# marcin-ochman/modular-slam

Measured on AMD Instinct MI355X. Metric: ORB keypoints extracted+matched /sec, 640×480 RGB-D, 1/2/4/8 GPU; HBM GB/s vs roofline, higher is better.
Workload: dtype u8

## Files before the change

modular-slam_amd/csrc/k_fast.hip:

```cpp
#include <type_traits>
#include "common.hpp"
#include "arc_score.hpp"

namespace mslam
{

constexpr int kTileP = 80;
constexpr int kTileX = 1;
constexpr int kScP = 68;

__device__ __forceinline__ CellDesc load_cell(const CellDesc* __restrict__ cells, int cell)
{
    typedef uint32_t u32x4_t __attribute__((ext_vector_type(4)));
    u32x4_t r;
    const uint32_t off = (uint32_t)cell * (uint32_t)sizeof(CellDesc);
    asm volatile("s_load_dwordx4 %0, %1, %2\n\ts_waitcnt lgkmcnt(0)" : "=s"(r) : "s"(cells), "s"(off));
    CellDesc c;
    c.level = (int16_t)(r.x & 0xFFFFu), c.cw = (int16_t)(r.x >> 16);
    c.ch = (int16_t)(r.y & 0xFFFFu), c.pad = 0;
    c.x0 = (int16_t)(r.z & 0xFFFFu), c.y0 = (int16_t)(r.z >> 16);
    c.ox = (int16_t)(r.w & 0xFFFFu), c.oy = (int16_t)(r.w >> 16);
    return c;
}
static_assert(sizeof(CellDesc) == 16, "load_cell reads a descriptor as four dwords");

__device__ __forceinline__ int min3i(int a, int b, int c) { return min(min(a, b), c); }
__device__ __forceinline__ int max3i(int a, int b, int c) { return max(max(a, b), c); }

__global__ __launch_bounds__(256) __attribute__((amdgpu_waves_per_eu(8, 8))) void k_fast_cells(const uint8_t* __restrict__ pyr, Geometry g,
                                                    const CellDesc* __restrict__ cells, uint32_t* __restrict__ cell_cnt,
                                                    uint32_t* __restrict__ cell_kp, int ini_thr, int min_thr, int n_frames)
{
    __shared__ __attribute__((aligned(16))) uint8_t tile[70 * kTileP];
    __shared__ __attribute__((aligned(16))) uint8_t sc[(66 * kScP + 15) / 16 * 16];
    __shared__ __attribute__((aligned(4))) uint16_t cand[64 * 64];
    __shared__ uint32_t bitmap[64 * 2];
    constexpr uint32_t kPassCap = 512;
    __shared__ uint16_t plist[kPassCap];
    __shared__ uint32_t n_cand, n_pass;

    const bool spread = n_frames < 8;
    const int xcd = blockIdx.x & 7, cell_id = spread ? (int)blockIdx.x : (int)(blockIdx.x >> 3);
    const int f_local = spread ? (int)blockIdx.y : (int)blockIdx.y * 8 + xcd;
    if(f_local >= n_frames)
        return;
    const size_t frame = (size_t)f_local + g.frame0;
    const CellDesc c = load_cell(cells, cell_id);
    const LevelGeom& lv = g.lv[c.level];
    const int cw = c.cw, ch = c.ch;
    const int tid = threadIdx.x, lane = tid & 63, wave = tid >> 6;

    {
        const uint8_t* src = pyr + frame * g.slab + lv.offset + (size_t)c.y0 * lv.pitch + (c.x0 - kTileX);
        const int n_chunks = ch * 5;
#pragma unroll
        for(int p = 0; p < 2; ++p)
        {
            const int t = p * 256 + tid;
            if(t < n_chunks)
            {
                const int r = (t * 13108) >> 16, j = t - r * 5;
                const uint32_t off = (uint32_t)(r * lv.pitch + 16 * j);
                __builtin_amdgcn_global_load_lds(
                    (const __attribute__((address_space(1))) void*)(src + off),
                    (__attribute__((address_space(3))) void*)&tile[(p * 256 + wave * 64) * 16], 16, 0, 0);
            }
        }
    }
    if(tid < (66 * kScP + 15) / 16 - 256)
        reinterpret_cast<uint4*>(sc)[256 + tid] = make_uint4(0u, 0u, 0u, 0u);
    if(tid < 128)
        bitmap[tid] = 0;
    if(tid == 0)
        n_cand = 0, n_pass = 0;
    __builtin_amdgcn_s_waitcnt(0x0F70);
    __syncthreads();

    const uint32_t n_cand_lds = (uint32_t)(size_t)(__attribute__((address_space(3))) void*)(&n_cand);
    const uint32_t n_pass_lds = (uint32_t)(size_t)(__attribute__((address_space(3))) void*)(&n_pass);
    uint32_t total = 0;
    for(int pass = 0; pass < 2; ++pass)
    {
        const int thr = pass == 0 ? ini_thr : min_thr;

        {
            typedef __attribute__((address_space(3))) uint32_t* lds32_t;
            typedef __attribute__((address_space(3))) uint16_t* lds16_t;
            typedef uint32_t u32x4_t __attribute__((ext_vector_type(4)));
            typedef __attribute__((address_space(3))) u32x4_t* lds128_t;
            uint32_t t_op = threadIdx.x;
            asm volatile("" : "+v"(t_op));
            const uint32_t ln = t_op & 63u;
            const int wv = __builtin_amdgcn_readfirstlane((int)(t_op >> 6));
            const int ngrp = (cw - 6 + 3) >> 2;
            const int lg = ngrp > 8 ? 4 : ngrp > 4 ? 3 : ngrp > 2 ? 2 : ngrp > 1 ? 1 : 0;
            const int i4 = (int)(ln & ((1u << lg) - 1u)), sub = (int)(ln >> lg);
            const int rps = 64 >> lg;
            const int n_steps = (ch - 6 + rps - 1) >> (6 - lg);
            const int tq = min(max(thr, 0), 254);
            const uint32_t kb = (uint32_t)(256 - ((tq + 256) >> 1)) * 0x01010101u;
            const uint32_t kd = (uint32_t)(255 - ((254 - tq) >> 1)) * 0x01010101u;
            const int xl = 3 + 4 * i4;
            const int n_col = min(max(cw - 3 - xl, 0), 4);
            const uint32_t colmask = (uint32_t)(0x80808080ull >> (8 * (4 - n_col)));
            const uint32_t tile_lds = (uint32_t)(size_t)(__attribute__((address_space(3))) void*)tile;
            const uint32_t cand_lds = (uint32_t)(size_t)(__attribute__((address_space(3))) void*)cand;
            const uint32_t seg_lds = (uint32_t)(size_t)(__attribute__((address_space(3))) void*)sc + (uint32_t)wv * 1024u;
            int y = 3 + wv * rps + sub;
            uint32_t row = tile_lds + (uint32_t)((y - 3) * kTileP + 4 * i4);
            uint32_t yx = (uint32_t)((y << 8) | xl);
            uint32_t n_grp = 0;
            auto steps = [&](auto checked) {
                constexpr bool CHECKED = decltype(checked)::value;
#pragma unroll 1
                for(int st = wv; st < n_steps; st += 4, y += CHECKED ? 4 * rps : 0, row += (uint32_t)(4 * rps * kTileP), yx += (uint32_t)(4 * rps) << 8)
                {
                    uint32_t keep = 0;
                    if(!CHECKED || (colmask != 0 && y < ch - 3))
                    {
                        const lds32_t r = lds_ptr<lds32_t>(row);
                        const uint32_t d0 = r[60], d1 = r[61], d2 = r[62];
                        const uint32_t nC = ~d1, U = r[1], D = r[121];
                        const uint32_t Lf = __builtin_amdgcn_alignbyte(d1, d0, 1);
                        const uint32_t Rt = __builtin_amdgcn_alignbyte(d2, d1, 3);
                        const uint32_t q0 = __builtin_amdgcn_lerp(D, nC, 0u), q8 = __builtin_amdgcn_lerp(U, nC, 0u);
                        const uint32_t q4 = __builtin_amdgcn_lerp(Rt, nC, 0u), q12 = __builtin_amdgcn_lerp(Lf, nC, 0u);
                        const uint32_t br = (__builtin_amdgcn_lerp(q0, kb, 0u) | __builtin_amdgcn_lerp(q8, kb, 0u)) &
                                            (__builtin_amdgcn_lerp(q4, kb, 0u) | __builtin_amdgcn_lerp(q12, kb, 0u));
                        const uint32_t nd = (__builtin_amdgcn_lerp(q0, kd, 0u) & __builtin_amdgcn_lerp(q8, kd, 0u)) |
                                            (__builtin_amdgcn_lerp(q4, kd, 0u) & __builtin_amdgcn_lerp(q12, kd, 0u));
                        keep = (br | ~nd) & (CHECKED ? colmask : 0x80808080u);
                    }
                    const bool any = keep != 0;
                    const unsigned long long vote = __ballot(any);
                    if(any)
                        lds_ptr<lds32_t>(seg_lds)[n_grp + __builtin_amdgcn_mbcnt_hi((uint32_t)(vote >> 32), __builtin_amdgcn_mbcnt_lo((uint32_t)vote, 0u))] =
                            keep | yx;
                    n_grp += (uint32_t)__popcll(vote);
                }
            };
            if(cw == 70 && ch == 70)
                steps(std::false_type{});
            else
                steps(std::true_type{});
            for(uint32_t i0 = 0; i0 < n_grp; i0 += 64)
            {
                const uint32_t rec = i0 + ln < n_grp ? lds_ptr<lds32_t>(seg_lds)[i0 + ln] : 0u;
                const bool f0 = (rec & 0x80u) != 0, f1 = (rec & 0x8000u) != 0, f2 = (rec & 0x800000u) != 0, f3 = (int)rec < 0;
                const unsigned long long m0 = __ballot(f0), m1 = __ballot(f1), m2 = __ballot(f2), m3 = __ballot(f3);
                const uint32_t c0 = (uint32_t)__popcll(m0), c1 = (uint32_t)__popcll(m1), c2 = (uint32_t)__popcll(m2),
                               c3 = (uint32_t)__popcll(m3);
                uint32_t base;
                {
                    uint32_t got;
                    unsigned long long save;
                    const uint32_t add = c0 + c1 + c2 + c3;
                    asm volatile("s_mov_b64 %1, exec\n\t"
                                 "s_mov_b64 exec, 1\n\t"
                                 "ds_add_rtn_u32 %0, %2, %3\n\t"
                                 "s_waitcnt lgkmcnt(0)\n\t"
                                 "s_mov_b64 exec, %1"
                                 : "=&v"(got), "=&s"(save)
                                 : "v"(n_cand_lds), "v"(add)
                                 : "memory");
                    base = (uint32_t)__builtin_amdgcn_readfirstlane((int)got);
                }
                const uint32_t v = rec & 0x7F7Fu;
                uint32_t b2 = cand_lds + 2u * base;
                if(f0)
                    *lds_ptr<lds16_t>(b2 + 2u * __builtin_amdgcn_mbcnt_hi((uint32_t)(m0 >> 32), __builtin_amdgcn_mbcnt_lo((uint32_t)m0, 0u))) = (uint16_t)v;
                b2 += 2u * c0;
                if(f1)
                    *lds_ptr<lds16_t>(b2 + 2u * __builtin_amdgcn_mbcnt_hi((uint32_t)(m1 >> 32), __builtin_amdgcn_mbcnt_lo((uint32_t)m1, 0u))) = (uint16_t)(v + 1);
                b2 += 2u * c1;
                if(f2)
                    *lds_ptr<lds16_t>(b2 + 2u * __builtin_amdgcn_mbcnt_hi((uint32_t)(m2 >> 32), __builtin_amdgcn_mbcnt_lo((uint32_t)m2, 0u))) = (uint16_t)(v + 2);
                b2 += 2u * c2;
                if(f3)
                    *lds_ptr<lds16_t>(b2 + 2u * __builtin_amdgcn_mbcnt_hi((uint32_t)(m3 >> 32), __builtin_amdgcn_mbcnt_lo((uint32_t)m3, 0u))) = (uint16_t)(v + 3);
            }
            {
                uint32_t z = 0;
                asm volatile("" : "+v"(z));
                lds_ptr<lds128_t>(seg_lds)[ln] = u32x4_t{z, z, z, z};
            }
        }
        __syncthreads();
        const uint32_t n = n_cand;

        for(uint32_t j = tid; 2 * j < n; j += 256)
        {
            const uint32_t two = *reinterpret_cast<const uint32_t*>(&cand[2 * j]);
            const uint32_t ca = two & 0xFFFFu, cb = 2 * j + 1 < n ? two >> 16 : ca;
            const int ay = (int)(ca >> 8), ax = (int)(ca & 0xFF), by = (int)(cb >> 8), bx = (int)(cb & 0xFF);
            const uint8_t* pa = &tile[ay * kTileP + ax + kTileX];
            const uint8_t* pb = &tile[by * kTileP + bx + kTileX];
            typedef unsigned short u16x2_t __attribute__((ext_vector_type(2)));
            uint32_t e[16];
#define MSLAM_E(k, off)                                                                    \
    {                                                                                      \
        u16x2_t v2;                                                                        \
        v2.x = (unsigned short)pa[off];                                                    \
        v2.y = (unsigned short)pb[off];                                                    \
        e[k] = __builtin_bit_cast(uint32_t, v2);                                           \
    }
            MSLAM_E(0, 3 * kTileP);
            MSLAM_E(1, 3 * kTileP + 1);
            MSLAM_E(2, 2 * kTileP + 2);
            MSLAM_E(3, kTileP + 3);
            MSLAM_E(4, 3);
            MSLAM_E(5, -kTileP + 3);
            MSLAM_E(6, -2 * kTileP + 2);
            MSLAM_E(7, -3 * kTileP + 1);
            MSLAM_E(8, -3 * kTileP);
            MSLAM_E(9, -3 * kTileP - 1);
            MSLAM_E(10, -2 * kTileP - 2);
            MSLAM_E(11, -kTileP - 3);
            MSLAM_E(12, -3);
            MSLAM_E(13, kTileP - 3);
            MSLAM_E(14, 2 * kTileP - 2);
            MSLAM_E(15, 3 * kTileP - 1);
#undef MSLAM_E
            int sa, sb;
            arc_score2_raw(e, (int)pa[0], (int)pb[0], sa, sb);
            const bool pass_a = sa >= thr && sa > 0, pass_b = sb >= thr && sb > 0 && 2 * j + 1 < n;
            if(pass_a)
                sc[(ay - 2) * kScP + (ax - 2)] = (uint8_t)sa;
            if(pass_b)
                sc[(by - 2) * kScP + (bx - 2)] = (uint8_t)sb;
            const unsigned long long ma = __ballot(pass_a), mb = __ballot(pass_b);
            const uint32_t na = (uint32_t)__popcll(ma), nb = (uint32_t)__popcll(mb);
            if(na + nb != 0)
            {
                uint32_t got;
                unsigned long long save;
                const uint32_t add = na + nb;
                asm volatile("s_mov_b64 %1, exec\n\t"
                             "s_mov_b64 exec, 1\n\t"
                             "ds_add_rtn_u32 %0, %2, %3\n\t"
                             "s_waitcnt lgkmcnt(0)\n\t"
                             "s_mov_b64 exec, %1"
                             : "=&v"(got), "=&s"(save)
                             : "v"(n_pass_lds), "v"(add)
                             : "memory");
                const uint32_t base = (uint32_t)__builtin_amdgcn_readfirstlane((int)got);
                const uint32_t ia = base + __builtin_amdgcn_mbcnt_hi((uint32_t)(ma >> 32), __builtin_amdgcn_mbcnt_lo((uint32_t)ma, 0u));
                const uint32_t ib = base + na + __builtin_amdgcn_mbcnt_hi((uint32_t)(mb >> 32), __builtin_amdgcn_mbcnt_lo((uint32_t)mb, 0u));
                if(pass_a && ia < kPassCap)
                    plist[ia] = (uint16_t)ca;
                if(pass_b && ib < kPassCap)
                    plist[ib] = (uint16_t)cb;
            }
        }
        __syncthreads();

        const uint32_t np = n_pass;
        const bool short_list = np <= kPassCap;
        for(uint32_t i = tid; i < (short_list ? np : n); i += 256)
        {
            const uint32_t cxy = short_list ? plist[i] : cand[i];
            const int cy = (int)(cxy >> 8), cx = (int)(cxy & 0xFF);
            const uint8_t* q = &sc[(cy - 2) * kScP + (cx - 2)];
            const int s = q[0];
            if(s >= thr && s > 0)
            {
                const int m = max(max3i(q[-kScP - 1], q[-kScP], q[-kScP + 1]),
                                  max(max3i(q[-1], q[1], q[kScP - 1]), max(q[kScP], q[kScP + 1])));
                if(s > m)
                    atomicOr(&bitmap[(cy - 3) * 2 + ((cx - 3) >> 5)], 1u << ((cx - 3) & 31));
            }
        }
        __syncthreads();

        if(wave == 0)
        {
            const unsigned long long m = bitmap[lane * 2] | ((unsigned long long)bitmap[lane * 2 + 1] << 32);
            const uint32_t cnt = (uint32_t)__popcll(m);
            uint32_t inc = cnt;
            inc += (uint32_t)__builtin_amdgcn_update_dpp(0, (int)inc, 0x111, 0xF, 0xF, true);
            inc += (uint32_t)__builtin_amdgcn_update_dpp(0, (int)inc, 0x112, 0xF, 0xF, true);
            inc += (uint32_t)__builtin_amdgcn_update_dpp(0, (int)inc, 0x114, 0xF, 0xE, true);
            inc += (uint32_t)__builtin_amdgcn_update_dpp(0, (int)inc, 0x118, 0xF, 0xC, true);
            inc += (uint32_t)__builtin_amdgcn_update_dpp(0, (int)inc, 0x142, 0xA, 0xF, true);
            inc += (uint32_t)__builtin_amdgcn_update_dpp(0, (int)inc, 0x143, 0xC, 0xF, true);
            total = (uint32_t)__builtin_amdgcn_readlane((int)inc, 63);
            if(total != 0)
            {
                uint32_t* out = cell_kp + (frame * g.n_cells + cell_id) * (size_t)kCellCap;
                uint32_t pos = inc - cnt;
                unsigned long long rest = m;
                const int y = lane + 3;
                while(rest)
                {
                    const int bx = __ffsll((long long)rest) - 1;
                    rest &= rest - 1;
                    out[pos++] = pack_kp(bx + 3 + c.ox, y + c.oy, sc[(y - 2) * kScP + (bx + 3 - 2)]);
                }
            }
            if(lane == 0)
            {
                n_cand = total != 0 ? 0xFFFFFFFFu : 0u;
                n_pass = 0;
            }
        }
        __syncthreads();
        const bool done = n_cand != 0;
        __syncthreads();
        if(done || pass == 1)
            break;
    }
    if(tid == 0)
        cell_cnt[frame * g.n_cells + cell_id] = total;
}

__global__ void k_denorm_selfcheck(uint32_t* out)
{
    const uint32_t t = threadIdx.x;
    const uint32_t a = t | ((255u - t) << 16), b = ((t * 7u + 3u) & 255u) | (((t * 13u + 1u) & 255u) << 16), c = 1u | (254u << 16);
    const uint32_t mx = pk_max3(a, b, c), mn = pk_min3(a, b, c);
    auto lo = [](uint32_t x) { return x & 0xFFFFu; };
    auto hi = [](uint32_t x) { return x >> 16; };
    const bool ok = lo(mx) == max(max(lo(a), lo(b)), lo(c)) && hi(mx) == max(max(hi(a), hi(b)), hi(c)) &&
                    lo(mn) == min(min(lo(a), lo(b)), lo(c)) && hi(mn) == min(min(hi(a), hi(b)), hi(c));
    const unsigned long long all = __ballot(ok);
    if(t == 0)
        out[0] = all == ~0ull ? 1u : 0u;
}

void launch_denorm_selfcheck(uint32_t* d_out, hipStream_t s) { hipLaunchKernelGGL(k_denorm_selfcheck, dim3(1), dim3(64), 0, s, d_out); }

void launch_fast(const uint8_t* d_pyr, const Geometry& g, const CellDesc* d_cells, uint32_t* d_cell_cnt,
                 uint32_t* d_cell_kp, int ini_thr, int min_thr, int frame0, int n_frames, hipStream_t s)
{
    const dim3 grid = n_frames < 8 ? dim3((unsigned)g.n_cells, (unsigned)n_frames) : dim3(8u * (unsigned)g.n_cells, (unsigned)((n_frames + 7) / 8));
    Geometry gg = g;
    gg.frame0 = frame0;
    hipLaunchKernelGGL(k_fast_cells, grid, dim3(256), 0, s, d_pyr, gg, d_cells, d_cell_cnt, d_cell_kp, ini_thr, min_thr,
                       n_frames);
}

}
```

Baseline: 665.0 million.

## Pack LDS into one struct, merge init clears, and compact candidates with a DPP prefix scan

Places all shared arrays in a single struct so the score-map tail, bitmap and counters can be zeroed with one dword store per thread. It also asserts the total stays under 20 KB so eight workgroups fit per CU. Tile staging now uses scalar base addresses and a full-cell specialization, and the per-thread lane geometry is computed inside the specialized lambda. Candidate compaction replaces four ballots and mbcnt chains with a per-lane popcount plus a DPP inclusive scan and inline-asm masked 16-bit writes. This trims scalar and vector ALU work, but the hand-written exec and vcc assembly is fragile and relies on the row_bcast semantics of the DPP scan.

```diff
diff --git a/modular-slam_amd/csrc/k_fast.hip b/modular-slam_amd/csrc/k_fast.hip
--- a/modular-slam_amd/csrc/k_fast.hip
+++ b/modular-slam_amd/csrc/k_fast.hip
@@ -31,13 +31,27 @@
                                                     const CellDesc* __restrict__ cells, uint32_t* __restrict__ cell_cnt,
                                                     uint32_t* __restrict__ cell_kp, int ini_thr, int min_thr, int n_frames)
 {
-    __shared__ __attribute__((aligned(16))) uint8_t tile[70 * kTileP];
-    __shared__ __attribute__((aligned(16))) uint8_t sc[(66 * kScP + 15) / 16 * 16];
-    __shared__ __attribute__((aligned(4))) uint16_t cand[64 * 64];
-    __shared__ uint32_t bitmap[64 * 2];
     constexpr uint32_t kPassCap = 512;
-    __shared__ uint16_t plist[kPassCap];
-    __shared__ uint32_t n_cand, n_pass;
+    struct Smem
+    {
+        __attribute__((aligned(16))) uint16_t cand[64 * 64];
+        __attribute__((aligned(16))) uint8_t tile[70 * kTileP];
+        __attribute__((aligned(16))) uint8_t sc[(66 * kScP + 15) / 16 * 16];
+        uint32_t bitmap[64 * 2];
+        uint32_t n_cand, n_pass;
+        uint16_t plist[kPassCap];
+    };
+    __shared__ Smem sm;
+    auto& tile = sm.tile;
+    auto& sc = sm.sc;
+    auto& cand = sm.cand;
+    auto& bitmap = sm.bitmap;
+    auto& plist = sm.plist;
+    uint32_t& n_cand = sm.n_cand;
+    uint32_t& n_pass = sm.n_pass;
+    static_assert(offsetof(Smem, bitmap) == offsetof(Smem, sc) + sizeof(sm.sc) && offsetof(Smem, n_pass) + 4 == offsetof(Smem, plist),
+                  "the clear at the start runs from the score map's tail through the counters");
+    static_assert(sizeof(Smem) <= 20 * 1024, "8 workgroups per CU");
 
     const bool spread = n_frames < 8;
     const int xcd = blockIdx.x & 7, cell_id = spread ? (int)blockIdx.x : (int)(blockIdx.x >> 3);
@@ -48,31 +62,43 @@
     const CellDesc c = load_cell(cells, cell_id);
     const LevelGeom& lv = g.lv[c.level];
     const int cw = c.cw, ch = c.ch;
-    const int tid = threadIdx.x, lane = tid & 63, wave = tid >> 6;
-
+    const int tid = threadIdx.x, wave = __builtin_amdgcn_readfirstlane(tid >> 6);
+
+    const bool full = cw == 70 && ch == 70;
     {
-        const uint8_t* src = pyr + frame * g.slab + lv.offset + (size_t)c.y0 * lv.pitch + (c.x0 - kTileX);
-        const int n_chunks = ch * 5;
-#pragma unroll
-        for(int p = 0; p < 2; ++p)
-        {
-            const int t = p * 256 + tid;
-            if(t < n_chunks)
-            {
-                const int r = (t * 13108) >> 16, j = t - r * 5;
-                const uint32_t off = (uint32_t)(r * lv.pitch + 16 * j);
-                __builtin_amdgcn_global_load_lds(
-                    (const __attribute__((address_space(1))) void*)(src + off),
-                    (__attribute__((address_space(3))) void*)&tile[(p * 256 + wave * 64) * 16], 16, 0, 0);
-            }
-        }
+        int wv = wave;
+        asm volatile("" : "+s"(wv));
+        unsigned long long base = (unsigned long long)(pyr + frame * g.slab + lv.offset + (size_t)c.y0 * lv.pitch + (c.x0 - kTileX));
+        unsigned long long base2 = base + (unsigned long long)(51 * lv.pitch + 16);
+        asm volatile("" : "+s"(base), "+s"(base2));
+        const int wrap = lv.pitch - 5 * 16;
+        const int r = (tid * 13108) >> 16, j = tid - r * 5;
+        const uint32_t off = (uint32_t)(__mul24(r, wrap) + 16 * tid);
+        int j4 = j >> 2;
+        asm volatile("" : "+v"(j4));
+        const uint32_t off2 = (uint32_t)(__mul24(j4, wrap) + (int)off);
+        auto stage = [&](auto full_cell) {
+            constexpr bool FULL = decltype(full_cell)::value;
+            const int n_chunks = FULL ? 70 * 5 : ch * 5;
+            if(FULL || tid < n_chunks)
+                __builtin_amdgcn_global_load_lds((const __attribute__((address_space(1))) void*)((const uint8_t*)base + off),
+                                                 (__attribute__((address_space(3))) void*)&tile[(wv * 64) * 16], 16, 0, 0);
+            if(tid + 256 < n_chunks)
+                __builtin_amdgcn_global_load_lds((const __attribute__((address_space(1))) void*)((const uint8_t*)base2 + off2),
+                                                 (__attribute__((address_space(3))) void*)&tile[(256 + wv * 64) * 16], 16, 0, 0);
+        };
+        if(full)
+            stage(std::true_type{});
+        else
+            stage(std::false_type{});
     }
-    if(tid < (66 * kScP + 15) / 16 - 256)
-        reinterpret_cast<uint4*>(sc)[256 + tid] = make_uint4(0u, 0u, 0u, 0u);
-    if(tid < 128)
-        bitmap[tid] = 0;
-    if(tid == 0)
-        n_cand = 0, n_pass = 0;
+    {
+        constexpr uint32_t kClearFrom = 4096, kClearDwords = 256;
+        static_assert(offsetof(Smem, sc) + kClearFrom + 4 * kClearDwords >= offsetof(Smem, plist) &&
+                          offsetof(Smem, sc) + kClearFrom + 4 * kClearDwords <= sizeof(Smem),
+                      "one dword per thread reaches the counters and stays inside the block");
+        reinterpret_cast<uint32_t*>(sc + kClearFrom)[tid] = 0;
+    }
     __builtin_amdgcn_s_waitcnt(0x0F70);
     __syncthreads();
 
@@ -85,38 +111,53 @@
 
         {
             typedef __attribute__((address_space(3))) uint32_t* lds32_t;
-            typedef __attribute__((address_space(3))) uint16_t* lds16_t;
             typedef uint32_t u32x4_t __attribute__((ext_vector_type(4)));
             typedef __attribute__((address_space(3))) u32x4_t* lds128_t;
             uint32_t t_op = threadIdx.x;
             asm volatile("" : "+v"(t_op));
             const uint32_t ln = t_op & 63u;
-            const int wv = __builtin_amdgcn_readfirstlane((int)(t_op >> 6));
-            const int ngrp = (cw - 6 + 3) >> 2;
-            const int lg = ngrp > 8 ? 4 : ngrp > 4 ? 3 : ngrp > 2 ? 2 : ngrp > 1 ? 1 : 0;
-            const int i4 = (int)(ln & ((1u << lg) - 1u)), sub = (int)(ln >> lg);
-            const int rps = 64 >> lg;
-            const int n_steps = (ch - 6 + rps - 1) >> (6 - lg);
-            const int tq = min(max(thr, 0), 254);
+            int wv = wave;
+            asm volatile("" : "+s"(wv));
+            int tq = max(thr, 0);
+            asm volatile("" : "+s"(tq));
+            tq = min(tq, 254);
             const uint32_t kb = (uint32_t)(256 - ((tq + 256) >> 1)) * 0x01010101u;
             const uint32_t kd = (uint32_t)(255 - ((254 - tq) >> 1)) * 0x01010101u;
-            const int xl = 3 + 4 * i4;
-            const int n_col = min(max(cw - 3 - xl, 0), 4);
-            const uint32_t colmask = (uint32_t)(0x80808080ull >> (8 * (4 - n_col)));
             const uint32_t tile_lds = (uint32_t)(size_t)(__attribute__((address_space(3))) void*)tile;
             const uint32_t cand_lds = (uint32_t)(size_t)(__attribute__((address_space(3))) void*)cand;
             const uint32_t seg_lds = (uint32_t)(size_t)(__attribute__((address_space(3))) void*)sc + (uint32_t)wv * 1024u;
-            int y = 3 + wv * rps + sub;
-            uint32_t row = tile_lds + (uint32_t)((y - 3) * kTileP + 4 * i4);
-            uint32_t yx = (uint32_t)((y << 8) | xl);
             uint32_t n_grp = 0;
             auto steps = [&](auto checked) {
                 constexpr bool CHECKED = decltype(checked)::value;
+                const int cwv = CHECKED ? cw : 70, chv = CHECKED ? ch : 70;
+                const int ngrp = (cwv - 6 + 3) >> 2;
+                int lg = 4;
+                if constexpr(CHECKED)
+                {
+                    int lz = __clz(max(ngrp, 1) - 1);
+                    asm volatile("" : "+s"(lz));
+                    lg = min(32 - lz, 4);
+                }
+                const int i4 = (int)(ln & ((1u << lg) - 1u)), sub = (int)(ln >> lg);
+                const int rps = 64 >> lg;
+                const int n_steps = (chv - 6 + rps - 1) >> (6 - lg);
+                const int xl = 3 + 4 * i4;
+                const int n_col = min(max(cwv - 3 - xl, 0), 4);
+                const uint32_t colmask = (uint32_t)(0x80808080ull >> (8 * (4 - n_col)));
+                int y = 3 + wv * rps + sub;
+                uint32_t row = tile_lds + (uint32_t)((y - 3) * kTileP + 4 * i4);
+                uint32_t yx = (uint32_t)((y << 8) | xl);
+                if constexpr(!CHECKED)
+                {
+                    const uint32_t ln4 = ln << 2, sub16 = ln & 0x30u;
+                    row = ln4 + sub16 + (tile_lds + (uint32_t)(wv * 4 * kTileP));
+                    yx = ((sub16 << 4) | (ln4 & 0x3Cu)) + (uint32_t)(((3 + 4 * wv) << 8) | 3);
+                }
 #pragma unroll 1
                 for(int st = wv; st < n_steps; st += 4, y += CHECKED ? 4 * rps : 0, row += (uint32_t)(4 * rps * kTileP), yx += (uint32_t)(4 * rps) << 8)
                 {
                     uint32_t keep = 0;
-                    if(!CHECKED || (colmask != 0 && y < ch - 3))
+                    if(!CHECKED || (colmask != 0 && y < chv - 3))
                     {
                         const lds32_t r = lds_ptr<lds32_t>(row);
                         const uint32_t d0 = r[60], d1 = r[61], d2 = r[62];
@@ -139,45 +180,61 @@
                     n_grp += (uint32_t)__popcll(vote);
                 }
             };
-            if(cw == 70 && ch == 70)
+            if(full)
                 steps(std::false_type{});
             else
                 steps(std::true_type{});
             for(uint32_t i0 = 0; i0 < n_grp; i0 += 64)
             {
                 const uint32_t rec = i0 + ln < n_grp ? lds_ptr<lds32_t>(seg_lds)[i0 + ln] : 0u;
-                const bool f0 = (rec & 0x80u) != 0, f1 = (rec & 0x8000u) != 0, f2 = (rec & 0x800000u) != 0, f3 = (int)rec < 0;
-                const unsigned long long m0 = __ballot(f0), m1 = __ballot(f1), m2 = __ballot(f2), m3 = __ballot(f3);
-                const uint32_t c0 = (uint32_t)__popcll(m0), c1 = (uint32_t)__popcll(m1), c2 = (uint32_t)__popcll(m2),
-                               c3 = (uint32_t)__popcll(m3);
+                const uint32_t cnt = (uint32_t)__popc(rec & 0x80808080u);
+                uint32_t inc = cnt;
+                inc += (uint32_t)__builtin_amdgcn_update_dpp(0, (int)inc, 0x111, 0xF, 0xF, true);
+                inc += (uint32_t)__builtin_amdgcn_update_dpp(0, (int)inc, 0x112, 0xF, 0xF, true);
+                inc += (uint32_t)__builtin_amdgcn_update_dpp(0, (int)inc, 0x114, 0xF, 0xE, true);
+                inc += (uint32_t)__builtin_amdgcn_update_dpp(0, (int)inc, 0x118, 0xF, 0xC, true);
+                inc += (uint32_t)__builtin_amdgcn_update_dpp(0, (int)inc, 0x142, 0xA, 0xF, true);
+                inc += (uint32_t)__builtin_amdgcn_update_dpp(0, (int)inc, 0x143, 0xC, 0xF, true);
                 uint32_t base;
                 {
                     uint32_t got;
                     unsigned long long save;
-                    const uint32_t add = c0 + c1 + c2 + c3;
                     asm volatile("s_mov_b64 %1, exec\n\t"
-                                 "s_mov_b64 exec, 1\n\t"
+                                 "s_lshl_b64 exec, 1, 63\n\t"
                                  "ds_add_rtn_u32 %0, %2, %3\n\t"
                                  "s_waitcnt lgkmcnt(0)\n\t"
                                  "s_mov_b64 exec, %1"
                                  : "=&v"(got), "=&s"(save)
-                                 : "v"(n_cand_lds), "v"(add)
-                                 : "memory");
-                    base = (uint32_t)__builtin_amdgcn_readfirstlane((int)got);
+                                 : "v"(n_cand_lds), "v"(inc)
+                                 : "memory", "scc");
+                    base = (uint32_t)__builtin_amdgcn_readlane((int)got, 63);
                 }
-                const uint32_t v = rec & 0x7F7Fu;
-                uint32_t b2 = cand_lds + 2u * base;
-                if(f0)
-                    *lds_ptr<lds16_t>(b2 + 2u * __builtin_amdgcn_mbcnt_hi((uint32_t)(m0 >> 32), __builtin_amdgcn_mbcnt_lo((uint32_t)m0, 0u))) = (uint16_t)v;
-                b2 += 2u * c0;
-                if(f1)
-                    *lds_ptr<lds16_t>(b2 + 2u * __builtin_amdgcn_mbcnt_hi((uint32_t)(m1 >> 32), __builtin_amdgcn_mbcnt_lo((uint32_t)m1, 0u))) = (uint16_t)(v + 1);
-                b2 += 2u * c1;
-                if(f2)
-                    *lds_ptr<lds16_t>(b2 + 2u * __builtin_amdgcn_mbcnt_hi((uint32_t)(m2 >> 32), __builtin_amdgcn_mbcnt_lo((uint32_t)m2, 0u))) = (uint16_t)(v + 2);
-                b2 += 2u * c2;
-                if(f3)
-                    *lds_ptr<lds16_t>(b2 + 2u * __builtin_amdgcn_mbcnt_hi((uint32_t)(m3 >> 32), __builtin_amdgcn_mbcnt_lo((uint32_t)m3, 0u))) = (uint16_t)(v + 3);
+                const uint32_t v = rec & 0x7F7Fu, v1 = v + 1, v2 = v + 2, v3 = v + 3;
+                uint32_t slot = cand_lds + 2u * base + 2u * (inc - cnt);
+                const uint32_t rec8 = rec << 8;
+                unsigned long long save;
+                asm volatile("v_cmp_gt_i16 vcc, 0, %3\n\t"
+                             "s_and_saveexec_b64 %1, vcc\n\t"
+                             "ds_write_b16 %0, %4\n\t"
+                             "v_add_u32 %0, 2, %0\n\t"
+                             "s_mov_b64 exec, %1\n\t"
+                             "v_cmp_gt_i16 vcc, 0, %2\n\t"
+                             "s_and_saveexec_b64 %1, vcc\n\t"
+                             "ds_write_b16 %0, %5\n\t"
+                             "v_add_u32 %0, 2, %0\n\t"
+                             "s_mov_b64 exec, %1\n\t"
+                             "v_cmp_gt_i32 vcc, 0, %3\n\t"
+                             "s_and_saveexec_b64 %1, vcc\n\t"
+                             "ds_write_b16 %0, %6\n\t"
+                             "v_add_u32 %0, 2, %0\n\t"
+                             "s_mov_b64 exec, %1\n\t"
+                             "v_cmp_gt_i32 vcc, 0, %2\n\t"
+                             "s_and_saveexec_b64 %1, vcc\n\t"
+                             "ds_write_b16 %0, %7\n\t"
+                             "s_mov_b64 exec, %1"
+                             : "+v"(slot), "=&s"(save)
+                             : "v"(rec), "v"(rec8), "v"(v), "v"(v1), "v"(v2), "v"(v3)
+                             : "memory", "vcc", "scc");
             }
             {
                 uint32_t z = 0;
@@ -274,6 +331,8 @@
 
         if(wave == 0)
         {
+            int lane = tid & 63;
+            asm volatile("" : "+v"(lane));
             const unsigned long long m = bitmap[lane * 2] | ((unsigned long long)bitmap[lane * 2 + 1] << 32);
             const uint32_t cnt = (uint32_t)__popcll(m);
             uint32_t inc = cnt;
```

Result: no change. 673.2 million (median of 3 runs) (+1.2%).
